# LayerXcom/zero-chain

Measured on NVIDIA H100. Metric: g1_msm_mops_2^20, higher is better.
Workload: dtype u32-limb Montgomery (Fq 12x32, Fr 8x32), integer

## Files before the change

### zero_chain_b200/csrc/msm.cuh

```cuda
#pragma once
#include <cuda_runtime.h>
#include <stdint.h>
#include "curve.cuh"
#include "curve_coop.cuh"
#include "msm_accum.cuh"
#include "tma.cuh"

namespace zkmsm {

constexpr int TILE = 131072;
constexpr int SORT_THREADS = 1024;
constexpr int COARSE_THREADS = 256;
constexpr uint32_t DIGIT_ZERO = 0xffffffffu;

static __global__ void k_msm_digits(const uint32_t *__restrict__ scalars, uint32_t n, int c, int W,
                             uint32_t *__restrict__ digits, int *__restrict__ err) {
    __shared__ __align__(128) uint4 tile[256 * 2];
    __shared__ uint64_t bar;
    uint32_t i0 = blockIdx.x * blockDim.x, i = i0 + threadIdx.x;
    uint32_t ws = blockIdx.y;
    uint32_t cnt = n - i0 < blockDim.x ? n - i0 : blockDim.x;
    if (threadIdx.x == 0) zktma::mbar_init(&bar, 1);
    __syncthreads();
    if (threadIdx.x == 0) {
// ... 213 lines not shown
    if (threadIdx.x < nb) {
        size_t b = ((size_t)g << low) + threadIdx.x;
        sizes[b] = v;
        bucket_off[b] = r0 + excl;
        hist[threadIdx.x] = r0 + excl;
        off[threadIdx.x] = excl;
        if (threadIdx.x == nb - 1) off[nb] = excl + v;
    }
    if (cb == n_coarse - 1 && dom == (int)gridDim.y - 1 && threadIdx.x == 0) bucket_off[((size_t)g + 1) << low] = r1;
    __syncthreads();
    const uint32_t total = r1 - r0;
    if (total > (uint32_t)FINE_MAX_SEGMENTS * FINE_STAGE) {
        block_for_each<uint2, 4>(coarse_sorted + r0, total, [&](uint2 e, uint64_t) { sorted[atomicAdd(&hist[e.y & fmask], 1u)] = e.x; });
        return;
    }
    for (uint32_t lo = 0; lo < nb;) {
        const uint32_t base = off[lo];
        const int fit = __syncthreads_count(threadIdx.x >= lo && threadIdx.x < nb && off[threadIdx.x + 1] - base <= (uint32_t)FINE_STAGE);
        const uint32_t hi = lo + (fit > 0 ? (uint32_t)fit : 1u);
        const bool direct = fit == 0;
        block_for_each<uint2, 2>(coarse_sorted + r0, total, [&](uint2 e, uint64_t) {
            const uint32_t k = e.y & fmask;
            if (k >= lo && k < hi) {
                const uint32_t p = atomicAdd(&hist[k], 1u);
                if (direct) sorted[p] = e.x;
                else stage[p - r0 - base] = e.x;
            }
        });
        __syncthreads();
        if (!direct)
            for (uint32_t j = threadIdx.x, m = off[hi] - base; j < m; j += blockDim.x) sorted[r0 + base + j] = stage[j];
        __syncthreads();
        lo = hi;
    }
}

constexpr int SCAN_T = 256, SCAN_E = 8, SCAN_B = SCAN_T * SCAN_E;
template <bool TASKS>
__device__ __forceinline__ uint32_t scan_load(const uint32_t *in, size_t i, uint32_t task_len) {
    uint32_t v = in[i];
    if (!TASKS) return v;
    if (v == 0) return 0;
    uint32_t t = (v + task_len / 2) / task_len;
    return t ? t : 1;
}
static __global__ void k_pick_task_len(const uint32_t *__restrict__ total_entries, const uint32_t *__restrict__ sorted_entries, uint32_t *__restrict__ task_len,
                                       uint32_t capacity, unsigned long long *__restrict__ work_counter, unsigned long long *__restrict__ xyzz_counter) {
    task_len[1] = 0;
    uint32_t total = *total_entries;
    *work_counter += *sorted_entries;
    *xyzz_counter += total;
    uint32_t waves = (total + (uint32_t)TASK_LEN_MAX * capacity - 1) / ((uint32_t)TASK_LEN_MAX * capacity);
    if (waves < 2) waves = 2;
    uint32_t target = (uint32_t)(0.97f * (float)waves * (float)capacity);
    uint32_t t = (total + target - 1) / (target ? target : 1);
    if (t < (uint32_t)TASK_LEN_MIN) t = TASK_LEN_MIN;
    if (t > (uint32_t)TASK_LEN_MAX + 8) t = TASK_LEN_MAX + 8;
    *task_len = t;
}
template <bool TASKS>
__global__ void __launch_bounds__(SCAN_T) k_scan_block(const uint32_t *__restrict__ in, uint32_t *__restrict__ out,
                                                       uint32_t *__restrict__ block_sums, size_t n, const uint32_t *__restrict__ task_len_p) {
    __shared__ uint32_t wsum[SCAN_T / 32];
    const uint32_t task_len = TASKS ? *task_len_p : 1u;
    size_t base = (size_t)blockIdx.x * SCAN_B + (size_t)threadIdx.x * SCAN_E;
    uint32_t v[SCAN_E], s = 0;
#pragma unroll
    for (int k = 0; k < SCAN_E; k++) { v[k] = base + k < n ? scan_load<TASKS>(in, base + k, task_len) : 0; s += v[k]; }
    uint32_t inc = s;
#pragma unroll
    for (int o = 1; o < 32; o <<= 1) { uint32_t t = __shfl_up_sync(0xffffffffu, inc, o); if ((threadIdx.x & 31) >= o) inc += t; }
    if ((threadIdx.x & 31) == 31) wsum[threadIdx.x >> 5] = inc;
    __syncthreads();
    if (threadIdx.x < 32) {
        uint32_t w = threadIdx.x < SCAN_T / 32 ? wsum[threadIdx.x] : 0, wi = w;
#pragma unroll
        for (int o = 1; o < 32; o <<= 1) { uint32_t t = __shfl_up_sync(0xffffffffu, wi, o); if (threadIdx.x >= o) wi += t; }
        if (threadIdx.x < SCAN_T / 32) wsum[threadIdx.x] = wi - w;
        if (threadIdx.x == SCAN_T / 32 - 1 && block_sums) block_sums[blockIdx.x] = wi;
    }
    __syncthreads();
    uint32_t ex = inc - s + wsum[threadIdx.x >> 5];
#pragma unroll
    for (int k = 0; k < SCAN_E; k++) { if (base + k < n) out[base + k] = ex; ex += v[k]; }
}
static __global__ void k_scan_add(uint32_t *__restrict__ out, const uint32_t *__restrict__ block_off, size_t n) {
    size_t i = (size_t)blockIdx.x * SCAN_B + threadIdx.x;
    uint32_t o = block_off[blockIdx.x];
    for (int k = 0; k < SCAN_E; k++, i += SCAN_T) if (i < n) out[i] += o;
}
template <bool TASKS>
inline void exclusive_scan(const uint32_t *in, uint32_t *out, size_t n, uint32_t *scratch, cudaStream_t st, const uint32_t *task_len_p = nullptr) {
    size_t nb = (n + SCAN_B - 1) / SCAN_B;
    if (nb == 0) nb = 1;
    uint32_t *bs = scratch;
    k_scan_block<TASKS><<<(unsigned)nb, SCAN_T, 0, st>>>(in, out, bs, n, task_len_p);
    if (nb == 1) {
        cudaMemcpyAsync(out + n, bs, 4, cudaMemcpyDeviceToDevice, st);
        return;
    }
    uint32_t *bo = scratch + nb + 1;
    exclusive_scan<false>(bs, bo, nb, bo + nb + 2, st);
    k_scan_add<<<(unsigned)nb, SCAN_T, 0, st>>>(out, bo, n);
    cudaMemcpyAsync(out + n, bo + nb, 4, cudaMemcpyDeviceToDevice, st);
}

constexpr int LEN_BINS = 256, LEN_BLOCK = 1024;
__device__ __forceinline__ uint32_t task_len_of(const uint32_t *bucket_off, const uint32_t *task_off, uint32_t b, uint32_t &nt) {
    nt = task_off[b + 1] - task_off[b];
    if (!nt) return 0;
    uint32_t size = bucket_off[b + 1] - bucket_off[b], len = (size + nt - 1) / nt;
    return len < (uint32_t)LEN_BINS ? len : (uint32_t)LEN_BINS - 1;
}
static __global__ void __launch_bounds__(LEN_BLOCK) k_len_hist(const uint32_t *__restrict__ bucket_off, const uint32_t *__restrict__ task_off,
                                                              uint32_t n_buckets, uint32_t *__restrict__ ghist) {
    __shared__ uint32_t sh[LEN_BINS];
    if (threadIdx.x < LEN_BINS) sh[threadIdx.x] = 0;
    __syncthreads();
    uint32_t b = blockIdx.x * LEN_BLOCK + threadIdx.x, nt = 0;
    if (b < n_buckets) { uint32_t len = task_len_of(bucket_off, task_off, b, nt); if (nt) atomicAdd(&sh[len], nt); }
    __syncthreads();
    if (threadIdx.x < LEN_BINS && sh[threadIdx.x]) atomicAdd(&ghist[threadIdx.x], sh[threadIdx.x]);
}
static __global__ void __launch_bounds__(LEN_BINS) k_len_scan(uint32_t *__restrict__ ghist, uint32_t *__restrict__ cursor) {
    __shared__ uint32_t sh[LEN_BINS];
    sh[threadIdx.x] = ghist[LEN_BINS - 1 - threadIdx.x];
    __syncthreads();
    if (threadIdx.x == 0) { uint32_t run = 0; for (int i = 0; i < LEN_BINS; i++) { uint32_t v = sh[i]; sh[i] = run; run += v; } }
    __syncthreads();
    cursor[LEN_BINS - 1 - threadIdx.x] = sh[threadIdx.x];
    ghist[threadIdx.x] = 0;
}
static __global__ void __launch_bounds__(LEN_BLOCK) k_len_place(const uint32_t *__restrict__ bucket_off, const uint32_t *__restrict__ task_off,
                                                               uint32_t n_buckets, uint32_t *__restrict__ cursor, uint32_t *__restrict__ order) {
    __shared__ uint32_t cnt[LEN_BINS], base[LEN_BINS];
    if (threadIdx.x < LEN_BINS) cnt[threadIdx.x] = 0;
    __syncthreads();
    uint32_t b = blockIdx.x * LEN_BLOCK + threadIdx.x, nt = 0, len = 0, local = 0;
    if (b < n_buckets) { len = task_len_of(bucket_off, task_off, b, nt); if (nt) local = atomicAdd(&cnt[len], nt); }
    __syncthreads();
    if (threadIdx.x < LEN_BINS && cnt[threadIdx.x]) base[threadIdx.x] = atomicAdd(&cursor[threadIdx.x], cnt[threadIdx.x]);
    __syncthreads();
    if (nt) {
        uint32_t pos = base[len] + local, t0 = task_off[b];
        for (uint32_t s = 0; s < nt; s++) order[pos + s] = t0 + s;
    }
}

constexpr uint32_t COMB_SERIAL_MAX = 32;
template <class F>
__global__ void __launch_bounds__(128) k_combine_serial(const XYZZ<F> *__restrict__ partials, const uint32_t *__restrict__ task_off,
                                                        uint32_t n_buckets, XYZZ<F> *__restrict__ buckets,
                                                        uint32_t *__restrict__ heavy_list, uint32_t *__restrict__ heavy_count) {
    uint32_t b = blockIdx.x * blockDim.x + threadIdx.x;
    if (b >= n_buckets) return;
    uint32_t t0 = task_off[b], t1 = task_off[b + 1];
    if (t1 - t0 > COMB_SERIAL_MAX) { heavy_list[atomicAdd(heavy_count, 1u)] = b; return; }
    XYZZ<F> acc = XYZZ<F>::inf();
    if (t1 > t0) acc = partials[t0];
    for (uint32_t t = t0 + 1; t < t1; t++) acc.add(partials[t]);
    buckets[b] = acc;
}
template <class F>
__global__ void __launch_bounds__(128) k_combine_warp(const XYZZ<F> *__restrict__ partials, const uint32_t *__restrict__ task_off,
                                                      const uint32_t *__restrict__ heavy_list, const uint32_t *__restrict__ heavy_count,
                                                      XYZZ<F> *__restrict__ buckets) {
    extern __shared__ unsigned char smraw[];
    XYZZ<F> *sm = reinterpret_cast<XYZZ<F> *>(smraw) + (threadIdx.x >> 5) * 32;
    const uint32_t lane = threadIdx.x & 31, n_warps = (gridDim.x * blockDim.x) >> 5, n_heavy = *heavy_count;
    for (uint32_t i = (blockIdx.x * blockDim.x + threadIdx.x) >> 5; i < n_heavy; i += n_warps) {
        uint32_t b = heavy_list[i], t0 = task_off[b], t1 = task_off[b + 1];
        XYZZ<F> acc = XYZZ<F>::inf();
        for (uint32_t t = t0 + lane; t < t1; t += 32) acc.add(partials[t]);
        __syncwarp();
        sm[lane] = acc;
        __syncwarp();
        for (int o = 16; o > 0; o >>= 1) {
            if (lane < (uint32_t)o) { XYZZ<F> x = sm[lane]; x.add(sm[lane + o]); sm[lane] = x; }
            __syncwarp();
        }
        if (lane == 0) buckets[b] = sm[0];
    }
}

constexpr int RED_T = 128, RED_SLICE = 512;
#ifndef ZK_RC_GL
#define ZK_RC_GL 8
#endif
constexpr int RC_GL = ZK_RC_GL;
#ifndef ZK_RC_MINB
#define ZK_RC_MINB 2
#endif
template <class F>
__device__ __forceinline__ void warp_tree(XYZZ<F> *slot, XYZZ<F> &acc, uint32_t lane) {
    slot[lane] = acc;
    __syncwarp();
    for (int o = 16; o > 0; o >>= 1) {
        if (lane < o) { XYZZ<F> x = slot[lane]; x.add(slot[lane + o]); slot[lane] = x; }
        __syncwarp();
    }
    acc = slot[0];
}
template <class F>
__global__ void __launch_bounds__(RED_T) k_bit_sums(const XYZZ<F> *__restrict__ B, int N, int n_slices, int n_bits, int n_dom,
                                                    XYZZ<F> *__restrict__ part) {
    extern __shared__ unsigned char smraw[];
    uint32_t lane = threadIdx.x & 31;
    XYZZ<F> *slot = reinterpret_cast<XYZZ<F> *>(smraw) + (threadIdx.x >> 5) * 32;
    size_t gw = ((size_t)blockIdx.x * blockDim.x + threadIdx.x) >> 5;
    if (gw >= (size_t)n_slices * n_bits * n_dom) return;
    int slice = (int)(gw % n_slices), bit = (int)((gw / n_slices) % n_bits), dom = (int)(gw / ((size_t)n_slices * n_bits));
    const XYZZ<F> *p = B + (size_t)dom * N;
    uint32_t k0 = (uint32_t)slice * (RED_SLICE / 2), k1 = k0 + RED_SLICE / 2;
    XYZZ<F> acc = XYZZ<F>::inf();
    for (uint32_t k = k0 + lane; k < k1; k += 32) {
        uint32_t d = ((k >> bit) << (bit + 1)) | (1u << bit) | (k & ((1u << bit) - 1u));
        if (d <= (uint32_t)N) acc.add(p[d - 1]);
    }
    warp_tree(slot, acc, lane);
    if (lane == 0) part[((size_t)dom * n_bits + bit) * n_slices + slice] = acc;
}
template <class F>
__global__ void __launch_bounds__(RED_T) k_sum_points(const XYZZ<F> *__restrict__ P, int N, int n_groups, XYZZ<F> *__restrict__ out) {
    extern __shared__ unsigned char smraw[];
    uint32_t lane = threadIdx.x & 31;
    XYZZ<F> *slot = reinterpret_cast<XYZZ<F> *>(smraw) + (threadIdx.x >> 5) * 32;
    size_t g = ((size_t)blockIdx.x * blockDim.x + threadIdx.x) >> 5;
    if (g >= (size_t)n_groups) return;
    const XYZZ<F> *p = P + g * N;
    XYZZ<F> acc = XYZZ<F>::inf();
    for (int j = lane; j < N; j += 32) acc.add(p[j]);
    warp_tree(slot, acc, lane);
    if (lane == 0) out[g] = acc;
}
constexpr int FIN_WARPS = 10;
template <class F>
__global__ void __launch_bounds__(FIN_WARPS * 32) k_finish_bits(const XYZZ<F> *__restrict__ X, int n_bits, int n_dom, XYZZ<F> *__restrict__ R) {
    extern __shared__ unsigned char smraw[];
    XYZZ<F> *vals = reinterpret_cast<XYZZ<F> *>(smraw);
    const int dom = blockIdx.x, w = threadIdx.x >> 5, lane = threadIdx.x & 31;
    if (dom >= n_dom) return;
    if (threadIdx.x < 2 * FIN_WARPS) vals[threadIdx.x] = (int)threadIdx.x < n_bits ? X[(size_t)dom * n_bits + threadIdx.x] : XYZZ<F>::inf();
    __syncthreads();
    for (int s = 0; (1 << s) < n_bits; s++) {
        const int step = 1 << s, i = w * 2 * step;
        if (i + step < n_bits) {
            XYZZ<F> hi = vals[i + step], v = vals[i];
            for (int k = 0; k < step; k++) zkcoop::dbl(hi);
            zkcoop::add(v, hi);
            __syncwarp();
            if (lane == 0) vals[i] = v;
        }
        __syncthreads();
    }
    if (threadIdx.x == 0) R[dom] = vals[0];
}
template <class F>
__device__ __noinline__ void add_outline(XYZZ<F> &acc, const XYZZ<F> &o) { acc.add(o); }
template <class F, int GL>
__global__ void __launch_bounds__(RED_T, (sizeof(F) == sizeof(Fq) ? ZK_RC_MINB : 1)) k_rowcol_sums(const XYZZ<F> *__restrict__ B, int N, int s, int n_dom, XYZZ<F> *__restrict__ rc) {
    extern __shared__ unsigned char smraw[];
    const uint32_t lane = threadIdx.x & 31, sub = lane & (GL - 1);
    XYZZ<F> *slot = reinterpret_cast<XYZZ<F> *>(smraw) + (threadIdx.x >> 5) * 32;
    const int S = 1 << s, nr = N >> s, nc = S - 1;
    const size_t n_items = (size_t)n_dom * (nr + nc);
    size_t item = ((((size_t)blockIdx.x * blockDim.x + threadIdx.x) >> 5) * (32 / GL)) + (lane / GL);
    const bool live = item < n_items;
    int dom = 0, idx = 0;
    XYZZ<F> acc = XYZZ<F>::inf();
    if (live) {
        dom = (int)(item / (nr + nc)); idx = (int)(item % (nr + nc));
        const XYZZ<F> *p = B + (size_t)dom * N;
        if (idx < nr) {
            int hi = idx + 1;
            for (int lo = sub; lo < S; lo += GL) { int d = hi * S + lo; if (d <= N) add_outline(acc, p[d - 1]); }
        } else {
            int lo = idx - nr + 1;
            for (int hi = sub; hi <= nr; hi += GL) { int d = hi * S + lo; if (d <= N) add_outline(acc, p[d - 1]); }
        }
    }
    slot[lane] = acc;
    __syncwarp();
    for (int o = GL / 2; o > 0; o >>= 1) {
        if (sub < (uint32_t)o) { XYZZ<F> x = slot[lane]; add_outline(x, slot[lane + o]); slot[lane] = x; }
        __syncwarp();
    }
    if (live && sub == 0) {
        if (idx < nr) rc[((size_t)2 * dom) * nr + idx] = slot[lane]; else rc[((size_t)2 * dom + 1) * nr + (idx - nr)] = slot[lane];
    }
}
constexpr int RC_L1 = 16, RC_L2 = 8;
template <class F>
__global__ void __launch_bounds__(RED_T) k_rowcol_stage1(const XYZZ<F> *__restrict__ B, int N, int s, int n_dom, int P1, XYZZ<F> *__restrict__ t1) {
    const int S = 1 << s, nr = N >> s, nc = S - 1;
    const int P1r = (S + RC_L1 - 1) / RC_L1, P1c = (nr + 1 + RC_L1 - 1) / RC_L1;
    size_t id = (size_t)blockIdx.x * blockDim.x + threadIdx.x;
    const size_t n_row = (size_t)n_dom * nr * P1r, n_col = (size_t)n_dom * nc * P1c;
    if (id >= n_row + n_col) return;
    int dom, idx, k, which;
    if (id < n_row) { which = 0; k = (int)(id % P1r); size_t q = id / P1r; idx = (int)(q % nr); dom = (int)(q / nr); }
    else { id -= n_row; which = 1; k = (int)(id % P1c); size_t q = id / P1c; idx = (int)(q % nc); dom = (int)(q / nc); }
    const XYZZ<F> *p = B + (size_t)dom * N;
    XYZZ<F> acc = XYZZ<F>::inf();
    if (which == 0) {
        int hi = idx + 1, lo1 = (k + 1) * RC_L1 < S ? (k + 1) * RC_L1 : S;
        for (int lo = k * RC_L1; lo < lo1; lo++) { int d = hi * S + lo; if (d <= N) acc.add(p[d - 1]); }
    } else {
        int lo = idx + 1, h1 = (k + 1) * RC_L1 < nr + 1 ? (k + 1) * RC_L1 : nr + 1;
        for (int hi = k * RC_L1; hi < h1; hi++) { int d = hi * S + lo; if (d <= N) acc.add(p[d - 1]); }
    }
    t1[((size_t)(2 * dom + which) * nr + idx) * P1 + k] = acc;
}
template <class F>
__global__ void __launch_bounds__(RED_T) k_seg_sums(const XYZZ<F> *__restrict__ in, size_t n_groups, int P_in, int L, int P_out, XYZZ<F> *__restrict__ out) {
    size_t id = (size_t)blockIdx.x * blockDim.x + threadIdx.x;
    if (id >= n_groups * P_out) return;
    const size_t g = id / P_out; const int k = (int)(id % P_out);
    const XYZZ<F> *p = in + g * P_in;
    int j1 = (k + 1) * L < P_in ? (k + 1) * L : P_in;
    XYZZ<F> acc = XYZZ<F>::inf();
    for (int j = k * L; j < j1; j++) acc.add(p[j]);
    out[id] = acc;
}
template <class F>
__global__ void __launch_bounds__(128) k_join_rowcol(const XYZZ<F> *__restrict__ Rrc, int s, int n_dom, XYZZ<F> *__restrict__ R) {
    int dom = (blockIdx.x * blockDim.x + threadIdx.x) >> 5;
    if (dom >= n_dom) return;
    XYZZ<F> r = Rrc[2 * dom];
    for (int k = 0; k < s; k++) zkcoop::dbl(r);
    zkcoop::add(r, Rrc[2 * dom + 1]);
    if ((threadIdx.x & 31) == 0) R[dom] = r;
}

template <class F>
__global__ void __launch_bounds__(32) k_horner_windows(const XYZZ<F> *__restrict__ R, int W, int c, XYZZ<F> *__restrict__ out) {
    XYZZ<F> r = R[W - 1];
    for (int w = W - 2; w >= 0; w--) {
        for (int k = 0; k < c; k++) zkcoop::dbl(r);
        zkcoop::add(r, R[w]);
    }
    if (threadIdx.x == 0) out[0] = r;
}

constexpr int PRE_K = 4;
template <class F>
__global__ void __launch_bounds__(128) k_precompute(Affine<F> *__restrict__ tbl, uint32_t n, int c, int W) {
    uint32_t i0 = (blockIdx.x * blockDim.x + threadIdx.x) * PRE_K;
    if (i0 >= n) return;
    int m = n - i0 < PRE_K ? n - i0 : PRE_K;
    for (int w = 1; w < W; w++) {
        XYZZ<F> q[PRE_K];
        F pre[PRE_K];
        F accz = F::one();
        for (int k = 0; k < m; k++) {
            Affine<F> a = tbl[(size_t)(w - 1) * n + i0 + k];
            XYZZ<F> x = XYZZ<F>::dbl_affine(a);
            for (int d = 1; d < c; d++) x = x.dbl();
            q[k] = x;
            pre[k] = accz;
            if (!x.is_inf()) accz = accz * x.zzz;
        }
        F inv = accz.inverse();
        for (int k = m - 1; k >= 0; k--) {
            Affine<F> r;
            if (q[k].is_inf()) r = Affine<F>::inf();
            else {
                F zi = inv * pre[k];
                inv = inv * q[k].zzz;
                F zi2 = (zi * q[k].zz).sqr();
                r.x = q[k].x * zi2; r.y = q[k].y * zi;
            }
            tbl[(size_t)w * n + i0 + k] = r;
        }
    }
}

template <class F>
__global__ void k_to_affine(const XYZZ<F> *__restrict__ in, Affine<F> *__restrict__ out, int n) {
    int i = blockIdx.x * blockDim.x + threadIdx.x;
    if (i < n) out[i] = in[i].to_affine();
}

}
```

### zero_chain_b200/csrc/msm_affine_core.cuh

```cuda
#pragma once
#include "curve.cuh"

namespace zkmsm {

enum { PAIR_ADD = 0, PAIR_DBL = 1, PAIR_COPY0 = 2, PAIR_COPY1 = 3, PAIR_INF = 4 };

template <class F>
struct PairIO {
    const Affine<F> *pts;
    const uint32_t *sorted;
    ZK_DEV Affine<F> load(uint32_t i) const {
        Affine<F> p;
        if (sorted) {
            uint32_t code = sorted[i];
            p = pts[code & 0x7fffffffu];
            p.y = p.y.cneg(code >> 31);
        } else p = pts[i];
        return p;
    }
};

template <class F>
ZK_DEV int pair_classify(const Affine<F> &p0, const Affine<F> &p1, bool has1, F &den) {
    den = F::one();
    if (!has1 || p1.is_inf()) return PAIR_COPY0;
    if (p0.is_inf()) return PAIR_COPY1;
    if (p0.x == p1.x) {
        if (p0.y == p1.y) {
            den = p0.y.dbl();
            if (!den.is_zero()) return PAIR_DBL;
            den = F::one();
            return PAIR_INF;
        }
        return PAIR_INF;
    }
    den = p1.x - p0.x;
    return PAIR_ADD;
}
template <class F>
ZK_DEV Affine<F> pair_finish(int mode, const Affine<F> &p0, const Affine<F> &p1, const F &dinv) {
    if (mode == PAIR_COPY0) return p0;
    if (mode == PAIR_COPY1) return p1;
    if (mode == PAIR_INF) return Affine<F>::inf();
    F lam;
    if (mode == PAIR_DBL) { F xx = p0.x.sqr(); lam = (xx.dbl() + xx) * dinv; }
    else lam = (p1.y - p0.y) * dinv;
    Affine<F> r;
    r.x = lam.sqr() - p0.x - p1.x;
    r.y = lam * (p0.x - r.x) - p0.y;
    return r;
}

}
```

### zero_chain_b200/csrc/msm_batchaff.cuh

```cuda
#pragma once
#include <cuda_runtime.h>
#include <stdint.h>
#include "curve.cuh"
#include "msm_affine_core.cuh"
#include "msm_warp_scan.cuh"

namespace zkmsm {

constexpr int BA_T = 128;
constexpr int BA_K = 32;
constexpr int BA_MINB = 4;
constexpr int BA_MAX_LEVELS = 8;
constexpr int BA_INV_T = 512;
constexpr uint32_t BA_NONE = 0xffffffffu;

static __global__ void k_half_sizes(const uint32_t *__restrict__ off_in, uint32_t *__restrict__ sizes_out, uint32_t n_buckets) {
    uint32_t b = blockIdx.x * blockDim.x + threadIdx.x;
    if (b < n_buckets) sizes_out[b] = (off_in[b + 1] - off_in[b] + 1) >> 1;
}

template <class F>
__device__ __forceinline__ void ba_store_f(F *dst, const F &v) {
    const uint4 *s = reinterpret_cast<const uint4 *>(&v);
    uint4 *d = reinterpret_cast<uint4 *>(dst);
#pragma unroll
    for (int k = 0; k < (int)(sizeof(F) / 16); k++) d[k] = s[k];
}
template <class F>
__device__ __forceinline__ F ba_load_f(const F *src) {
    F v;
    const uint4 *s = reinterpret_cast<const uint4 *>(src);
    uint4 *d = reinterpret_cast<uint4 *>(&v);
#pragma unroll
    for (int k = 0; k < (int)(sizeof(F) / 16); k++) d[k] = s[k];
    return v;
}
template <class F>
__device__ __forceinline__ F ba_ldg_f(const F *src) {
    F v;
    const uint4 *s = reinterpret_cast<const uint4 *>(src);
    uint4 *d = reinterpret_cast<uint4 *>(&v);
#pragma unroll
    for (int k = 0; k < (int)(sizeof(F) / 16); k++) d[k] = __ldg(s + k);
    return v;
}
template <class F, bool FIRST>
__device__ __forceinline__ const F *ba_x(const F *in_x, uint32_t code) { return FIRST ? in_x + 2 * (size_t)(code & 0x7fffffffu) : in_x + code; }
template <class F, bool FIRST>
__device__ __forceinline__ const F *ba_y(const F *in_x, const F *in_y, uint32_t code) { return FIRST ? ba_x<F, FIRST>(in_x, code) + 1 : in_y + code; }
template <class F, bool FIRST>
__device__ __forceinline__ Affine<F> ba_load_point(const F *in_x, const F *in_y, uint32_t code) {
    Affine<F> p;
    p.x = ba_ldg_f(ba_x<F, FIRST>(in_x, code));
    p.y = ba_ldg_f(ba_y<F, FIRST>(in_x, in_y, code));
    if (FIRST) p.y = p.y.cneg(code >> 31);
    return p;
}

struct BaWalk {
    uint32_t b, out0, out1, in0, in1;
    __device__ __forceinline__ BaWalk(const uint32_t *off_in, const uint32_t *off_out, uint32_t n_buckets, uint32_t o) {
        uint32_t lo = 0, hi = n_buckets;
        while (hi - lo > 1) { uint32_t mid = (lo + hi) >> 1; if (off_out[mid] <= o) lo = mid; else hi = mid; }
        b = lo; out0 = off_out[b]; out1 = off_out[b + 1]; in0 = off_in[b]; in1 = off_in[b + 1];
    }
    __device__ __forceinline__ void forward(const uint32_t *off_in, const uint32_t *off_out, uint32_t o) {
        while (o >= out1) { b++; out0 = out1; out1 = off_out[b + 1]; in0 = in1; in1 = off_in[b + 1]; }
    }
    __device__ __forceinline__ void backward(const uint32_t *off_in, const uint32_t *off_out, uint32_t o) {
        while (o < out0) { b--; out1 = out0; out0 = off_out[b]; in1 = in0; in0 = off_in[b]; }
    }
    template <bool FIRST>
    __device__ __forceinline__ uint2 src(const uint32_t *sorted, uint32_t o) const {
        const uint32_t i0 = in0 + 2 * (o - out0);
        uint2 s;
        s.x = FIRST ? sorted[i0] : i0;
        s.y = i0 + 1 < in1 ? (FIRST ? sorted[i0 + 1] : i0 + 1) : BA_NONE;
        return s;
    }
};
__device__ __forceinline__ uint32_t ba_lane_first(size_t tid, int K) { return (uint32_t)(tid >> 5) * 32u * (uint32_t)K + (uint32_t)(tid & 31); }
__device__ __forceinline__ int ba_lane_count(uint32_t total, uint32_t oa, int K) {
    if (oa >= total) return 0;
    const uint32_t n = (total - oa + 31) >> 5;
    return n < (uint32_t)K ? (int)n : K;
}

template <class F, bool FIRST>
__global__ void __launch_bounds__(BA_T, 4) k_ba_forward(const F *__restrict__ in_x, const F *__restrict__ in_y, const uint32_t *__restrict__ sorted,
                                                         const uint32_t *__restrict__ off_in, const uint32_t *__restrict__ off_out, uint32_t n_buckets, int K,
                                                         F *__restrict__ prefix, F *__restrict__ block_totals) {
    const uint32_t total = off_out[n_buckets];
    const uint32_t n_blocks = (total + BA_T * K - 1) / (BA_T * K);
    if (blockIdx.x >= n_blocks) return;
    const int t = threadIdx.x;
    const size_t T_total = (size_t)gridDim.x * BA_T, tid = (size_t)blockIdx.x * BA_T + t;
    const uint32_t oa = ba_lane_first(tid, K);
    const int n = ba_lane_count(total, oa, K);
    F run = F::one();
    if (n > 0) {
        BaWalk w(off_in, off_out, n_buckets, oa);
        uint2 s0 = w.src<FIRST>(sorted, oa), s1 = make_uint2(0, BA_NONE);
        F xa0 = ba_ldg_f(ba_x<F, FIRST>(in_x, s0.x)), xa1 = s0.y != BA_NONE ? ba_ldg_f(ba_x<F, FIRST>(in_x, s0.y)) : F::zero();
        F xb0 = F::zero(), xb1 = F::zero();
        if (n > 1) {
            w.forward(off_in, off_out, oa + 32);
            s1 = w.src<FIRST>(sorted, oa + 32);
            xb0 = ba_ldg_f(ba_x<F, FIRST>(in_x, s1.x));
            if (s1.y != BA_NONE) xb1 = ba_ldg_f(ba_x<F, FIRST>(in_x, s1.y));
        }
        for (int k = 0; k < n; k++) {
            const uint2 cur = s0;
            const F x0 = xa0, x1 = xa1;
            s0 = s1; xa0 = xb0; xa1 = xb1;
            if (k + 2 < n) {
                const uint32_t o = oa + 32u * (uint32_t)(k + 2);
                w.forward(off_in, off_out, o);
                s1 = w.src<FIRST>(sorted, o);
                xb0 = ba_ldg_f(ba_x<F, FIRST>(in_x, s1.x));
                if (s1.y != BA_NONE) xb1 = ba_ldg_f(ba_x<F, FIRST>(in_x, s1.y));
            }
            ba_store_f(prefix + (size_t)k * T_total + tid, run);
            if (cur.y == BA_NONE) continue;
            F den = x1 - x0;
            if (den.is_zero() || x0.is_zero() || x1.is_zero()) {
                Affine<F> p0 = ba_load_point<F, FIRST>(in_x, in_y, cur.x), p1 = ba_load_point<F, FIRST>(in_x, in_y, cur.y);
                if (pair_classify(p0, p1, true, den) > PAIR_DBL) continue;
            }
            run = run * den;
        }
    }
    F others, all;
    ba_warp_products(run, others, all);
    ba_store_f(prefix + (size_t)K * T_total + tid, others);
    if ((t & 31) == 0) ba_store_f(block_totals + (tid >> 5), all);
}

template <class F>
__global__ void __launch_bounds__(BA_INV_T) k_ba_invert(const F *__restrict__ totals, const uint32_t *__restrict__ off_out, uint32_t n_buckets, int K,
                                                        F *__restrict__ scratch, F *__restrict__ inv_out) {
    extern __shared__ unsigned char ba_smem[];
    F *node = reinterpret_cast<F *>(ba_smem);
    const uint32_t total = off_out[n_buckets];
    const uint32_t n = ((total + BA_T * K - 1) / (BA_T * K)) * (BA_T / 32);
    const int t = threadIdx.x;
    const uint32_t per = (n + BA_INV_T - 1) / BA_INV_T, c0 = t * per, c1 = c0 + per < n ? c0 + per : n;
    F run = F::one();
    for (uint32_t i = c0; i < c1; i++) { ba_store_f(scratch + i, run); run = run * ba_load_f(totals + i); }
    node[BA_INV_T + t] = run;
    for (int s = BA_INV_T / 2; s >= 1; s >>= 1) {
        __syncthreads();
        if (t < s) node[s + t] = node[2 * (s + t)] * node[2 * (s + t) + 1];
    }
    __syncthreads();
    if (t == 0) node[1] = node[1].inverse();
    for (int s = 1; s < BA_INV_T; s <<= 1) {
        __syncthreads();
        if (t < s) {
            F inv = node[s + t], l = node[2 * (s + t)], r = node[2 * (s + t) + 1];
            node[2 * (s + t)] = inv * r;
            node[2 * (s + t) + 1] = inv * l;
        }
    }
    __syncthreads();
    F inv = node[BA_INV_T + t];
    for (uint32_t i = c1; i-- > c0;) {
        F v = ba_load_f(totals + i);
        ba_store_f(inv_out + i, inv * ba_load_f(scratch + i));
        inv = inv * v;
    }
}

template <class F, bool FIRST, int MINB>
__global__ void __launch_bounds__(BA_T, MINB) k_ba_backward(const F *__restrict__ in_x, const F *__restrict__ in_y, const uint32_t *__restrict__ sorted,
                                                             const uint32_t *__restrict__ off_in, const uint32_t *__restrict__ off_out, uint32_t n_buckets, int K,
                                                             const F *__restrict__ prefix, const F *__restrict__ block_inv,
                                                             F *__restrict__ out_x, F *__restrict__ out_y) {
    constexpr int PV = (int)(sizeof(Affine<F>) / 16), FV = (int)(sizeof(F) / 16);
    extern __shared__ unsigned char ba_smem[];
    uint4 *stage = reinterpret_cast<uint4 *>(ba_smem);
    const uint32_t total = off_out[n_buckets];
    const uint32_t n_blocks = (total + BA_T * K - 1) / (BA_T * K);
    if (blockIdx.x >= n_blocks) return;
    const int t = threadIdx.x;
    const size_t T_total = (size_t)gridDim.x * BA_T, tid = (size_t)blockIdx.x * BA_T + t;
    const uint32_t oa = ba_lane_first(tid, K);
    const int n = ba_lane_count(total, oa, K);
    if (n == 0) return;
    F inv = ba_load_f(block_inv + (tid >> 5)) * ba_load_f(prefix + (size_t)K * T_total + tid);
    uint4 *slot = stage + t;
    auto copy = [&](int v, const F *src) {
        const uint4 *s = reinterpret_cast<const uint4 *>(src);
#pragma unroll
        for (int u = 0; u < FV; u++)
            asm volatile("cp.async.cg.shared.global [%0], [%1], 16;" ::"r"((uint32_t)__cvta_generic_to_shared(slot + (v + u) * BA_T)), "l"(s + u) : "memory");
    };
    auto prefetch = [&](int k, uint2 src) {
        const uint32_t c1 = src.y == BA_NONE ? src.x : src.y;
        copy(0, ba_x<F, FIRST>(in_x, src.x));
        copy(FV, ba_y<F, FIRST>(in_x, in_y, src.x));
        copy(PV, ba_x<F, FIRST>(in_x, c1));
        copy(PV + FV, ba_y<F, FIRST>(in_x, in_y, c1));
        copy(2 * PV, prefix + (size_t)k * T_total + tid);
        asm volatile("cp.async.commit_group;" ::: "memory");
    };
    BaWalk w(off_in, off_out, n_buckets, oa + 32u * (uint32_t)(n - 1));
    uint2 src = w.src<FIRST>(sorted, oa + 32u * (uint32_t)(n - 1));
    prefetch(n - 1, src);
    for (int k = n; k-- > 0;) {
        asm volatile("cp.async.wait_group 0;" ::: "memory");
        Affine<F> p0, p1;
        F pre;
        {
            uint4 *d0 = reinterpret_cast<uint4 *>(&p0), *d1 = reinterpret_cast<uint4 *>(&p1), *d2 = reinterpret_cast<uint4 *>(&pre);
#pragma unroll
            for (int v = 0; v < PV; v++) { d0[v] = slot[v * BA_T]; d1[v] = slot[(PV + v) * BA_T]; }
#pragma unroll
            for (int v = 0; v < FV; v++) d2[v] = slot[(2 * PV + v) * BA_T];
        }
        const uint2 cur = src;
        if (k > 0) {
            const uint32_t o = oa + 32u * (uint32_t)(k - 1);
            w.backward(off_in, off_out, o);
            src = w.src<FIRST>(sorted, o);
            prefetch(k - 1, src);
        }
        const bool has1 = cur.y != BA_NONE;
        if (FIRST) { p0.y = p0.y.cneg(cur.x >> 31); if (has1) p1.y = p1.y.cneg(cur.y >> 31); }
        if (!has1) p1 = Affine<F>::inf();
        F den;
        const int mode = pair_classify(p0, p1, has1, den);
        F dinv = F::one();
        if (mode <= PAIR_DBL) { dinv = inv * pre; inv = inv * den; }
        Affine<F> r = pair_finish(mode, p0, p1, dinv);
        const uint32_t o = oa + 32u * (uint32_t)k;
        ba_store_f(out_x + o, r.x);
        ba_store_f(out_y + o, r.y);
    }
}

template <class F> constexpr size_t ba_smem_forward() { return 0; }
template <class F> constexpr size_t ba_smem_backward() { return (size_t)BA_T * (2 * sizeof(Affine<F>) + sizeof(F)); }
template <class F> constexpr size_t ba_smem_invert() { return 2 * BA_INV_T * sizeof(F); }

}
```

### zero_chain_b200/csrc/msm_driver.cuh

```cuda
#pragma once
#include "internal.h"
#include "msm.cuh"
#include "msm_batchaff.cuh"
#include "codec.cuh"
#include <stdlib.h>

namespace zkmsm {

template <class F>
int build_tables_t(zk_ctx *ctx, zk_bases *b) {
    unsigned thr = 128, blk = (unsigned)((b->n + thr * PRE_K - 1) / (thr * PRE_K));
    k_precompute<F><<<blk, thr, 0, ctx->stream>>>((Affine<F> *)b->d_tbl, (uint32_t)b->n, b->c, b->W);
    ZK_CUDA(cudaGetLastError());
    return ZK_OK;
}

template <class F>
int msm_run_t(zk_ctx *ctx, const zk_bases *b, const uint32_t *d_scalars, size_t n, size_t batch) {
    cudaStream_t st = ctx->stream;
    const int c = b->c, W = b->W, nbins = 1 << (c - 1);
    const bool tables = b->tables;
    if (!tables && batch != 1) { zk_set_error("batched MSM needs precomputed tables"); return ZK_ERR_INVALID; }
    const size_t n_dom = tables ? batch : (size_t)W;
    const uint64_t e_dom = tables ? (uint64_t)n * W : (uint64_t)n;
    const size_t E = (size_t)n * W * batch;
    if (E >= ((size_t)1 << 31)) { zk_set_error("MSM too large for 31-bit entry payloads (n*W*batch = %zu)", E); return ZK_ERR_INVALID; }
    const bool two_level = c > 16;
    const int low = two_level ? (c - 1) - 9 : 0, sort_bins = two_level ? 512 : nbins;
    size_t smem = (size_t)sort_bins * 4;
    uint32_t tile_len = TILE;
    if (two_level) {
        int per_sm = 0;
        ZK_CUDA(cudaOccupancyMaxActiveBlocksPerMultiprocessor(&per_sm, k_coarse_scatter, COARSE_THREADS, 0));
        tile_len = coarse_tile_len(e_dom, n_dom, per_sm * ctx->sm_count);
    }
    const int tiles = (int)((e_dom + tile_len - 1) / tile_len);
    const size_t NB = n_dom * nbins;
    size_t t_max = E / TASK_LEN_MAX + 2 * (size_t)ctx->sm_count * 1024u + 1;
    t_max += NB + 1;
    const size_t pt = sizeof(XYZZ<F>);
    ZK_TRY(ctx->digits.reserve(E * 4));
    ZK_TRY(ctx->tile_hist.reserve(n_dom * tiles * (size_t)(c > 16 ? 512 : nbins) * 4));
    ZK_TRY(ctx->tile_off.reserve(n_dom * tiles * (size_t)(c > 16 ? 512 : nbins) * 4));
    ZK_TRY(ctx->sizes.reserve((NB + 1) * 4));
    ZK_TRY(ctx->bucket_off.reserve((NB + 1) * 4));
    ZK_TRY(ctx->task_off.reserve((NB + 1) * 4));
    ZK_TRY(ctx->scan_scratch.reserve((2 * (NB / SCAN_B + 8) + 4096) * 4));
    ZK_TRY(ctx->sorted.reserve(E * 4));
    ZK_TRY(ctx->partials.reserve(t_max * pt));
    ZK_TRY(ctx->buckets.reserve(NB * pt));
    const int n_bits = c;
    const int n_slices = (nbins / 2 + RED_SLICE / 2 - 1) / (RED_SLICE / 2) > 0 ? (nbins / 2 + RED_SLICE / 2 - 1) / (RED_SLICE / 2) : 1;
    ZK_TRY(ctx->red_part.reserve(2 * n_dom * n_bits * (size_t)n_slices * pt));
    ZK_TRY(ctx->red_x.reserve(2 * n_dom * n_bits * pt));
    ZK_TRY(ctx->result.reserve((n_dom + batch + 1) * pt));

    uint32_t *digits = ctx->digits.as<uint32_t>();
    {
        dim3 g((unsigned)((n + 255) / 256), (unsigned)batch);
        k_msm_digits<<<g, 256, 0, st>>>(d_scalars, (uint32_t)n, c, W, digits, ctx->d_err);
    }
    const size_t SB = n_dom * (size_t)sort_bins;
    if (smem > 48 * 1024) {
        ZK_CUDA(cudaFuncSetAttribute(k_tile_hist, cudaFuncAttributeMaxDynamicSharedMemorySize, (int)smem));
        ZK_CUDA(cudaFuncSetAttribute(k_scatter, cudaFuncAttributeMaxDynamicSharedMemorySize, (int)smem));
    }
    dim3 gs((unsigned)tiles, (unsigned)n_dom);
    if (!two_level) {
        k_tile_hist<<<gs, SORT_THREADS, smem, st>>>(digits, e_dom, nbins, 0, ctx->tile_hist.as<uint32_t>(), tiles, tile_len, false);
        k_col_scan<<<(unsigned)((NB + 255) / 256), 256, 0, st>>>(ctx->tile_hist.as<uint32_t>(), ctx->tile_off.as<uint32_t>(), ctx->sizes.as<uint32_t>(),
                                                                nbins, tiles, (int)n_dom);
        exclusive_scan<false>(ctx->sizes.as<uint32_t>(), ctx->bucket_off.as<uint32_t>(), NB, ctx->scan_scratch.as<uint32_t>(), st);
        k_scatter<<<gs, SORT_THREADS, smem, st>>>(digits, e_dom, nbins, ctx->tile_off.as<uint32_t>(), ctx->bucket_off.as<uint32_t>(),
                                                  ctx->sorted.as<uint32_t>(), tiles, tile_len);
    } else {
        ZK_TRY(ctx->sorted2.reserve(E * sizeof(uint2)));
        ZK_TRY(ctx->coarse_off.reserve((SB + 1) * 4)); ZK_TRY(ctx->coarse_sizes.reserve((SB + 1) * 4));
        k_tile_hist<<<gs, COARSE_THREADS, smem, st>>>(digits, e_dom, sort_bins, low, ctx->tile_hist.as<uint32_t>(), tiles, tile_len, true);
        k_bin_scan<<<(unsigned)SB, COARSE_THREADS, 0, st>>>(ctx->tile_hist.as<uint32_t>(), ctx->tile_off.as<uint32_t>(), ctx->coarse_sizes.as<uint32_t>(), tiles);
        exclusive_scan<false>(ctx->coarse_sizes.as<uint32_t>(), ctx->coarse_off.as<uint32_t>(), SB, ctx->scan_scratch.as<uint32_t>(), st);
        k_coarse_scatter<<<gs, COARSE_THREADS, 0, st>>>(digits, e_dom, low, ctx->tile_off.as<uint32_t>(), ctx->coarse_off.as<uint32_t>(),
                                                        ctx->sorted2.as<uint2>(), tiles, tile_len);
        ZK_CUDA(cudaFuncSetAttribute(k_fine_sort, cudaFuncAttributeMaxDynamicSharedMemorySize, FINE_STAGE * 4));
        k_fine_sort<<<dim3(512, (unsigned)n_dom), 1024, FINE_STAGE * 4, st>>>(ctx->sorted2.as<uint2>(), ctx->coarse_off.as<uint32_t>(), 512, low,
                                                                 ctx->sizes.as<uint32_t>(), ctx->bucket_off.as<uint32_t>(), ctx->sorted.as<uint32_t>());
    }
    const F *cur_x = (const F *)b->d_tbl, *cur_y = nullptr;
    const uint32_t *cur_sorted = ctx->sorted.as<uint32_t>(), *cur_off = ctx->bucket_off.as<uint32_t>(), *cur_sizes = ctx->sizes.as<uint32_t>();
    struct ProfPair {
        cudaEvent_t a = nullptr, b = nullptr; bool kept = false;
        ~ProfPair() { if (!kept) { if (a) cudaEventDestroy(a); if (b) cudaEventDestroy(b); } }
    } prof;
    cudaEvent_t &ev0 = prof.a, &ev1 = prof.b;
    {
        int levels = 0;
        if (ctx->opts.ba_min_entries >= 0 && (long)E >= ctx->opts.ba_min_entries) {
            if (ctx->opts.ba_levels >= 0) levels = (int)(ctx->opts.ba_levels < BA_MAX_LEVELS ? ctx->opts.ba_levels : BA_MAX_LEVELS);
            else for (size_t avg = E / NB; avg >= 12 && levels < BA_MAX_LEVELS; avg >>= 1) levels++;
        }
        if (ctx->prof_on && levels > 0) { cudaEventCreate(&ev0); cudaEventCreate(&ev1); cudaEventRecord(ev0, st); }
        size_t in_max = E;
        int minb = BA_MINB, k_force = 0;
        (void)minb;
#ifdef ZK_EXPERIMENTS
        if (const char *e = getenv("ZK_BA_MINB")) minb = atoi(e);
        if (const char *e = getenv("ZK_BA_K")) k_force = atoi(e);
#endif
        DevBuf *pts_buf[2] = {&ctx->aff_pts0, &ctx->aff_pts1}, *off_buf[2] = {&ctx->aff_off0, &ctx->aff_off1}, *sz_buf[2] = {&ctx->aff_sizes0, &ctx->aff_sizes1};
        if (levels > 0) {
            if (ba_smem_backward<F>() > 48 * 1024) {
                ZK_CUDA(cudaFuncSetAttribute(k_ba_backward<F, true, BA_MINB>, cudaFuncAttributeMaxDynamicSharedMemorySize, (int)ba_smem_backward<F>()));
                ZK_CUDA(cudaFuncSetAttribute(k_ba_backward<F, false, BA_MINB>, cudaFuncAttributeMaxDynamicSharedMemorySize, (int)ba_smem_backward<F>()));
#ifdef ZK_EXPERIMENTS
                ZK_CUDA(cudaFuncSetAttribute(k_ba_backward<F, true, 3>, cudaFuncAttributeMaxDynamicSharedMemorySize, (int)ba_smem_backward<F>()));
                ZK_CUDA(cudaFuncSetAttribute(k_ba_backward<F, false, 3>, cudaFuncAttributeMaxDynamicSharedMemorySize, (int)ba_smem_backward<F>()));
#endif
            }
            if (ba_smem_invert<F>() > 48 * 1024)
                ZK_CUDA(cudaFuncSetAttribute(k_ba_invert<F>, cudaFuncAttributeMaxDynamicSharedMemorySize, (int)ba_smem_invert<F>()));
        }
        for (int l = 0; l < levels; l++) {
            const size_t out_max = (in_max + NB) / 2 + 1;
            int K = BA_K;
            if (k_force > 0) K = k_force;
            const unsigned grid = (unsigned)((out_max + (size_t)BA_T * K - 1) / ((size_t)BA_T * K));
            const size_t T_total = (size_t)grid * BA_T;
            DevBuf *pts_o = pts_buf[l & 1], *off_o = off_buf[l & 1], *sz_o = sz_buf[l & 1];
            ZK_TRY(pts_o->reserve(out_max * sizeof(Affine<F>)));
            F *out_x = pts_o->as<F>(), *out_y = out_x + out_max;
            ZK_TRY(off_o->reserve((NB + 1) * 4)); ZK_TRY(sz_o->reserve((NB + 1) * 4));
            ZK_TRY(ctx->aff_scratch.reserve((size_t)(K + 1) * T_total * sizeof(F)));
            const size_t n_tot = (size_t)grid * (BA_T / 32);
            ZK_TRY(ctx->aff_tot.reserve(3 * n_tot * sizeof(F)));
            F *tot = ctx->aff_tot.as<F>(), *tot_scr = tot + n_tot, *tot_inv = tot + 2 * n_tot;
            k_half_sizes<<<(unsigned)((NB + 255) / 256), 256, 0, st>>>(cur_off, sz_o->as<uint32_t>(), (uint32_t)NB);
            exclusive_scan<false>(sz_o->as<uint32_t>(), off_o->as<uint32_t>(), NB, ctx->scan_scratch.as<uint32_t>(), st);
            const uint32_t *off_out = off_o->as<uint32_t>();
            if (l == 0)
                k_ba_forward<F, true><<<grid, BA_T, ba_smem_forward<F>(), st>>>(cur_x, cur_y, cur_sorted, cur_off, off_out, (uint32_t)NB, K, ctx->aff_scratch.as<F>(), tot);
            else
                k_ba_forward<F, false><<<grid, BA_T, ba_smem_forward<F>(), st>>>(cur_x, cur_y, nullptr, cur_off, off_out, (uint32_t)NB, K, ctx->aff_scratch.as<F>(), tot);
            k_ba_invert<F><<<1, BA_INV_T, ba_smem_invert<F>(), st>>>(tot, off_out, (uint32_t)NB, K, tot_scr, tot_inv);
            const int Kb = K;
#define ZK_BA_BWD(FIRST_, MB_) k_ba_backward<F, FIRST_, MB_><<<grid, BA_T, ba_smem_backward<F>(), st>>>(cur_x, cur_y, cur_sorted, cur_off, off_out, (uint32_t)NB, Kb, \
                                                                                                    ctx->aff_scratch.as<F>(), tot_inv, out_x, out_y)
#ifdef ZK_EXPERIMENTS
            if (minb == 3) { if (l == 0) ZK_BA_BWD(true, 3); else ZK_BA_BWD(false, 3); } else
#endif
            { if (l == 0) ZK_BA_BWD(true, BA_MINB); else ZK_BA_BWD(false, BA_MINB); }
#undef ZK_BA_BWD
            cur_x = out_x; cur_y = out_y; cur_sorted = nullptr;
            cur_off = off_out; cur_sizes = sz_o->as<uint32_t>();
            in_max = out_max;
        }
    }
    uint32_t *d_task_len = (uint32_t *)(ctx->d_err + 8);
    const uint32_t capacity = (uint32_t)ctx->sm_count * 3u * 128u;
    unsigned long long *d_work = (unsigned long long *)(ctx->d_err + (sizeof(F) == sizeof(Fq) ? 10 : 12));
    k_pick_task_len<<<1, 1, 0, st>>>(cur_off + NB, ctx->bucket_off.as<uint32_t>() + NB, d_task_len, capacity, d_work, d_work + 2);
    exclusive_scan<true>(cur_sizes, ctx->task_off.as<uint32_t>(), NB, ctx->scan_scratch.as<uint32_t>(), st, d_task_len);
    XYZZ<F> *partials = ctx->partials.as<XYZZ<F>>(), *buckets = ctx->buckets.as<XYZZ<F>>();
    const uint32_t *order = nullptr;
    {
        bool want = E / NB < 256;
        if (want) {
            ZK_TRY(ctx->task_order.reserve(t_max * 4)); ZK_TRY(ctx->len_hist.reserve(2 * LEN_BINS * 4 + 64));
            uint32_t *gh = ctx->len_hist.as<uint32_t>(), *cur = gh + LEN_BINS;
            if (!ctx->len_hist_zeroed) { ZK_CUDA(cudaMemsetAsync(gh, 0, 2 * LEN_BINS * 4, st)); ctx->len_hist_zeroed = true; }
            unsigned nb = (unsigned)((NB + LEN_BLOCK - 1) / LEN_BLOCK);
            k_len_hist<<<nb, LEN_BLOCK, 0, st>>>(cur_off, ctx->task_off.as<uint32_t>(), (uint32_t)NB, gh);
            k_len_scan<<<1, LEN_BINS, 0, st>>>(gh, cur);
            k_len_place<<<nb, LEN_BLOCK, 0, st>>>(cur_off, ctx->task_off.as<uint32_t>(), (uint32_t)NB, cur, ctx->task_order.as<uint32_t>());
            order = ctx->task_order.as<uint32_t>();
        }
    }
    {
        const uint32_t *so = cur_sorted, *bo = cur_off, *to = ctx->task_off.as<uint32_t>();
        unsigned grid = (unsigned)((t_max + 127) / 128);
        if (ctx->prof_on && !ev0) { cudaEventCreate(&ev0); cudaEventCreate(&ev1); cudaEventRecord(ev0, st); }
        k_accumulate<F, 3><<<grid, 128, 0, st>>>(cur_x, cur_y, so, bo, to, (uint32_t)NB, order, partials);
    }
    if (ctx->prof_on) { cudaEventRecord(ev1, st); ctx->prof_events.push_back(ev0); ctx->prof_events.push_back(ev1); prof.kept = true; }
    if (ctx->split_tail) {
        ZK_CUDA(cudaEventRecord(ctx->ev_front, st));
        ZK_CUDA(cudaStreamWaitEvent(ctx->tail, ctx->ev_front, 0));
        st = ctx->tail;
    }
    const size_t sm_warp = 4 * 32 * pt;
    if (sm_warp > 48 * 1024) {
        ZK_CUDA(cudaFuncSetAttribute(k_combine_warp<F>, cudaFuncAttributeMaxDynamicSharedMemorySize, (int)sm_warp));
        ZK_CUDA(cudaFuncSetAttribute(k_bit_sums<F>, cudaFuncAttributeMaxDynamicSharedMemorySize, (int)sm_warp));
        ZK_CUDA(cudaFuncSetAttribute(k_sum_points<F>, cudaFuncAttributeMaxDynamicSharedMemorySize, (int)sm_warp));
        ZK_CUDA(cudaFuncSetAttribute(k_finish_bits<F>, cudaFuncAttributeMaxDynamicSharedMemorySize, (int)sm_warp));
    }
    ZK_TRY(ctx->heavy_list.reserve((NB + 1) * 4));
    uint32_t *heavy_count = d_task_len + 1;
    k_combine_serial<F><<<(unsigned)((NB + 127) / 128), 128, 0, st>>>(partials, ctx->task_off.as<uint32_t>(), (uint32_t)NB, buckets,
                                                                      ctx->heavy_list.as<uint32_t>(), heavy_count);
    k_combine_warp<F><<<(unsigned)(2 * ctx->sm_count), 128, sm_warp, st>>>(partials, ctx->task_off.as<uint32_t>(), ctx->heavy_list.as<uint32_t>(), heavy_count, buckets);
    XYZZ<F> *part = ctx->red_part.as<XYZZ<F>>(), *X = ctx->red_x.as<XYZZ<F>>(), *R = ctx->result.as<XYZZ<F>>();
    auto bit_reduce = [&](const XYZZ<F> *Bk, int N, int bits, size_t nd, XYZZ<F> *out) {
        int slices = (N / 2 + RED_SLICE / 2 - 1) / (RED_SLICE / 2); if (slices < 1) slices = 1;
        size_t n_w = (size_t)slices * bits * nd, n_g = nd * (size_t)bits;
        k_bit_sums<F><<<(unsigned)((n_w * 32 + RED_T - 1) / RED_T), RED_T, sm_warp, st>>>(Bk, N, slices, bits, (int)nd, part);
        k_sum_points<F><<<(unsigned)((n_g * 32 + RED_T - 1) / RED_T), RED_T, sm_warp, st>>>(part, slices, (int)n_g, X);
        k_finish_bits<F><<<(unsigned)nd, FIN_WARPS * 32, 2 * FIN_WARPS * sizeof(XYZZ<F>), st>>>(X, bits, (int)nd, out);
    };
    XYZZ<F> *Rdom = tables ? R : R + 1;
    if ((n_dom >= 8 && c >= 7) || (tables && c > 16)) {
        const int s = (c - 1) / 2, nr = nbins >> s, nc = (1 << s) - 1;
        ZK_TRY(ctx->red_rows.reserve(2 * n_dom * (size_t)nr * pt));
        ZK_TRY(ctx->result.reserve((3 * n_dom + batch + 4) * pt));
        R = ctx->result.as<XYZZ<F>>();
        Rdom = tables ? R : R + 1;
        XYZZ<F> *rc = ctx->red_rows.as<XYZZ<F>>(), *Rrc = R + n_dom + 2;
        if (sm_warp > 48 * 1024) {
            ZK_CUDA(cudaFuncSetAttribute(k_rowcol_sums<F, RC_GL>, cudaFuncAttributeMaxDynamicSharedMemorySize, (int)sm_warp));
        }
        size_t n_items = n_dom * (size_t)(nr + nc);
        if (n_dom >= 8) {
            ZK_CUDA(cudaMemsetAsync(rc, 0, 2 * n_dom * (size_t)nr * pt, st));
            constexpr int per_warp = 32 / RC_GL;
            k_rowcol_sums<F, RC_GL><<<(unsigned)((((n_items + per_warp - 1) / per_warp) * 32 + RED_T - 1) / RED_T), RED_T, sm_warp, st>>>(buckets, nbins, s, (int)n_dom, rc);
        } else {
            const size_t n_slots = 2 * n_dom * (size_t)nr;
            const int longest = (1 << s) > nr + 1 ? (1 << s) : nr + 1;
            const int P1 = (longest + RC_L1 - 1) / RC_L1, P2 = (P1 + RC_L2 - 1) / RC_L2;
            ZK_TRY(ctx->red_tmp.reserve(n_slots * (size_t)(P1 + P2) * pt));
            XYZZ<F> *t1 = ctx->red_tmp.as<XYZZ<F>>(), *t2 = t1 + n_slots * P1;
            const int P1r = ((1 << s) + RC_L1 - 1) / RC_L1, P1c = (nr + 1 + RC_L1 - 1) / RC_L1;
            const size_t live = n_dom * ((size_t)nr * P1r + (size_t)nc * P1c);
            ZK_CUDA(cudaMemsetAsync(t1, 0, n_slots * (size_t)P1 * pt, st));
            k_rowcol_stage1<F><<<(unsigned)((live + RED_T - 1) / RED_T), RED_T, 0, st>>>(buckets, nbins, s, (int)n_dom, P1, t1);
            k_seg_sums<F><<<(unsigned)((n_slots * P2 + RED_T - 1) / RED_T), RED_T, 0, st>>>(t1, n_slots, P1, RC_L2, P2, t2);
            k_seg_sums<F><<<(unsigned)((n_slots + RED_T - 1) / RED_T), RED_T, 0, st>>>(t2, n_slots, P2, P2, 1, rc);
        }
        bit_reduce(rc, nr, c - s, 2 * n_dom, Rrc);
        k_join_rowcol<F><<<(unsigned)((n_dom * 32 + 127) / 128), 128, 0, st>>>(Rrc, s, (int)n_dom, Rdom);
    } else {
        bit_reduce(buckets, nbins, n_bits, n_dom, Rdom);
    }
    if (!tables) k_horner_windows<F><<<1, 32, 0, st>>>(Rdom, W, c, R);
    ZK_CUDA(cudaGetLastError());
    return ZK_OK;
}

template <class F>
int encode_results_t(zk_ctx *ctx, size_t count, int compressed, uint8_t *d_out) {
    zkcodec::k_encode_xyzz<F><<<(unsigned)((count + 31) / 32), 32, 0, ctx->stream>>>(ctx->result.as<XYZZ<F>>(), (int)count, compressed, d_out);
    ZK_CUDA(cudaGetLastError());
    return ZK_OK;
}

}
```

Before: 165.6.

## Park pair source indices in forward pass for Fq batch-affine backward

For the Fq field, the forward batch-affine kernel now saves each step's source-index pair to scratch. The backward kernel reads these pairs directly instead of re-walking bucket offsets and re-reading the sorted array, and prefetches one step ahead. pair_finish for Fq also moves the doubling numerator into a noinline cold helper and merges the two lambda multiplies to cut code size and register pressure. The row/col stage1 loop is unified into a single strided loop. The cost is extra scratch memory and additional global stores and loads of uint2 per step.

```diff
diff --git a/zero_chain_b200/csrc/msm.cuh b/zero_chain_b200/csrc/msm.cuh
--- a/zero_chain_b200/csrc/msm.cuh
+++ b/zero_chain_b200/csrc/msm.cuh
@@ -539,13 +539,10 @@
     else { id -= n_row; which = 1; k = (int)(id % P1c); size_t q = id / P1c; idx = (int)(q % nc); dom = (int)(q / nc); }
     const XYZZ<F> *p = B + (size_t)dom * N;
     XYZZ<F> acc = XYZZ<F>::inf();
-    if (which == 0) {
-        int hi = idx + 1, lo1 = (k + 1) * RC_L1 < S ? (k + 1) * RC_L1 : S;
-        for (int lo = k * RC_L1; lo < lo1; lo++) { int d = hi * S + lo; if (d <= N) acc.add(p[d - 1]); }
-    } else {
-        int lo = idx + 1, h1 = (k + 1) * RC_L1 < nr + 1 ? (k + 1) * RC_L1 : nr + 1;
-        for (int hi = k * RC_L1; hi < h1; hi++) { int d = hi * S + lo; if (d <= N) acc.add(p[d - 1]); }
-    }
+    int d, step, m;
+    if (which == 0) { const int lo0 = k * RC_L1, lo1 = lo0 + RC_L1 < S ? lo0 + RC_L1 : S; d = (idx + 1) * S + lo0; step = 1; m = lo1 - lo0; }
+    else { const int h0 = k * RC_L1, h1 = h0 + RC_L1 < nr + 1 ? h0 + RC_L1 : nr + 1; d = h0 * S + idx + 1; step = S; m = h1 - h0; }
+    for (int j = 0; j < m; j++, d += step) if (d <= N) acc.add(p[d - 1]);
     t1[((size_t)(2 * dom + which) * nr + idx) * P1 + k] = acc;
 }
 template <class F>
diff --git a/zero_chain_b200/csrc/msm_affine_core.cuh b/zero_chain_b200/csrc/msm_affine_core.cuh
--- a/zero_chain_b200/csrc/msm_affine_core.cuh
+++ b/zero_chain_b200/csrc/msm_affine_core.cuh
@@ -37,13 +37,21 @@
     den = p1.x - p0.x;
     return PAIR_ADD;
 }
+#ifdef ZK_HOST_EMUL
+#define ZK_PAIR_COLD inline
+#else
+#define ZK_PAIR_COLD __device__ __noinline__
+#endif
+template <class F>
+ZK_PAIR_COLD F pair_dbl_num(const F x) { F xx = x.sqr(); return xx.dbl() + xx; }
 template <class F>
 ZK_DEV Affine<F> pair_finish(int mode, const Affine<F> &p0, const Affine<F> &p1, const F &dinv) {
     if (mode == PAIR_COPY0) return p0;
     if (mode == PAIR_COPY1) return p1;
     if (mode == PAIR_INF) return Affine<F>::inf();
     F lam;
-    if (mode == PAIR_DBL) { F xx = p0.x.sqr(); lam = (xx.dbl() + xx) * dinv; }
+    if (sizeof(F) == sizeof(Fq)) lam = (mode == PAIR_DBL ? pair_dbl_num(p0.x) : p1.y - p0.y) * dinv;
+    else if (mode == PAIR_DBL) { F xx = p0.x.sqr(); lam = (xx.dbl() + xx) * dinv; }
     else lam = (p1.y - p0.y) * dinv;
     Affine<F> r;
     r.x = lam.sqr() - p0.x - p1.x;
diff --git a/zero_chain_b200/csrc/msm_batchaff.cuh b/zero_chain_b200/csrc/msm_batchaff.cuh
--- a/zero_chain_b200/csrc/msm_batchaff.cuh
+++ b/zero_chain_b200/csrc/msm_batchaff.cuh
@@ -79,6 +79,8 @@
         return s;
     }
 };
+template <class F> __host__ __device__ constexpr bool ba_parks_pairs() { return sizeof(F) == sizeof(Fq); }
+
 __device__ __forceinline__ uint32_t ba_lane_first(size_t tid, int K) { return (uint32_t)(tid >> 5) * 32u * (uint32_t)K + (uint32_t)(tid & 31); }
 __device__ __forceinline__ int ba_lane_count(uint32_t total, uint32_t oa, int K) {
     if (oa >= total) return 0;
@@ -89,7 +91,7 @@
 template <class F, bool FIRST>
 __global__ void __launch_bounds__(BA_T, 4) k_ba_forward(const F *__restrict__ in_x, const F *__restrict__ in_y, const uint32_t *__restrict__ sorted,
                                                          const uint32_t *__restrict__ off_in, const uint32_t *__restrict__ off_out, uint32_t n_buckets, int K,
-                                                         F *__restrict__ prefix, F *__restrict__ block_totals) {
+                                                         F *__restrict__ prefix, uint2 *__restrict__ srcs, F *__restrict__ block_totals) {
     const uint32_t total = off_out[n_buckets];
     const uint32_t n_blocks = (total + BA_T * K - 1) / (BA_T * K);
     if (blockIdx.x >= n_blocks) return;
@@ -121,6 +123,7 @@
                 if (s1.y != BA_NONE) xb1 = ba_ldg_f(ba_x<F, FIRST>(in_x, s1.y));
             }
             ba_store_f(prefix + (size_t)k * T_total + tid, run);
+            if (ba_parks_pairs<F>()) srcs[(size_t)k * T_total + tid] = cur;
             if (cur.y == BA_NONE) continue;
             F den = x1 - x0;
             if (den.is_zero() || x0.is_zero() || x1.is_zero()) {
@@ -173,7 +176,8 @@
 
 template <class F, bool FIRST, int MINB>
 __global__ void __launch_bounds__(BA_T, MINB) k_ba_backward(const F *__restrict__ in_x, const F *__restrict__ in_y, const uint32_t *__restrict__ sorted,
-                                                             const uint32_t *__restrict__ off_in, const uint32_t *__restrict__ off_out, uint32_t n_buckets, int K,
+                                                             const uint2 *__restrict__ srcs, const uint32_t *__restrict__ off_in,
+                                                             const uint32_t *__restrict__ off_out, uint32_t n_buckets, int K,
                                                              const F *__restrict__ prefix, const F *__restrict__ block_inv,
                                                              F *__restrict__ out_x, F *__restrict__ out_y) {
     constexpr int PV = (int)(sizeof(Affine<F>) / 16), FV = (int)(sizeof(F) / 16);
@@ -204,9 +208,17 @@
         copy(2 * PV, prefix + (size_t)k * T_total + tid);
         asm volatile("cp.async.commit_group;" ::: "memory");
     };
+    constexpr bool PARKED = ba_parks_pairs<F>();
     BaWalk w(off_in, off_out, n_buckets, oa + 32u * (uint32_t)(n - 1));
-    uint2 src = w.src<FIRST>(sorted, oa + 32u * (uint32_t)(n - 1));
+    auto pair_of = [&](int k) -> uint2 {
+        if (PARKED) return srcs[(size_t)k * T_total + tid];
+        const uint32_t o = oa + 32u * (uint32_t)k;
+        w.backward(off_in, off_out, o);
+        return w.src<FIRST>(sorted, o);
+    };
+    uint2 src = pair_of(n - 1), nxt = src;
     prefetch(n - 1, src);
+    if (PARKED && n > 1) nxt = pair_of(n - 2);
     for (int k = n; k-- > 0;) {
         asm volatile("cp.async.wait_group 0;" ::: "memory");
         Affine<F> p0, p1;
@@ -220,10 +232,10 @@
         }
         const uint2 cur = src;
         if (k > 0) {
-            const uint32_t o = oa + 32u * (uint32_t)(k - 1);
-            w.backward(off_in, off_out, o);
-            src = w.src<FIRST>(sorted, o);
-            prefetch(k - 1, src);
+            if (!PARKED) nxt = pair_of(k - 1);
+            prefetch(k - 1, nxt);
+            src = nxt;
+            if (PARKED && k > 1) nxt = pair_of(k - 2);
         }
         const bool has1 = cur.y != BA_NONE;
         if (FIRST) { p0.y = p0.y.cneg(cur.x >> 31); if (has1) p1.y = p1.y.cneg(cur.y >> 31); }
diff --git a/zero_chain_b200/csrc/msm_driver.cuh b/zero_chain_b200/csrc/msm_driver.cuh
--- a/zero_chain_b200/csrc/msm_driver.cuh
+++ b/zero_chain_b200/csrc/msm_driver.cuh
@@ -129,7 +129,8 @@
             ZK_TRY(pts_o->reserve(out_max * sizeof(Affine<F>)));
             F *out_x = pts_o->as<F>(), *out_y = out_x + out_max;
             ZK_TRY(off_o->reserve((NB + 1) * 4)); ZK_TRY(sz_o->reserve((NB + 1) * 4));
-            ZK_TRY(ctx->aff_scratch.reserve((size_t)(K + 1) * T_total * sizeof(F)));
+            ZK_TRY(ctx->aff_scratch.reserve((size_t)(K + 1) * T_total * sizeof(F) + (ba_parks_pairs<F>() ? (size_t)K * T_total * sizeof(uint2) : 0)));
+            uint2 *srcs = reinterpret_cast<uint2 *>(ctx->aff_scratch.as<F>() + (size_t)(K + 1) * T_total);
             const size_t n_tot = (size_t)grid * (BA_T / 32);
             ZK_TRY(ctx->aff_tot.reserve(3 * n_tot * sizeof(F)));
             F *tot = ctx->aff_tot.as<F>(), *tot_scr = tot + n_tot, *tot_inv = tot + 2 * n_tot;
@@ -137,12 +138,12 @@
             exclusive_scan<false>(sz_o->as<uint32_t>(), off_o->as<uint32_t>(), NB, ctx->scan_scratch.as<uint32_t>(), st);
             const uint32_t *off_out = off_o->as<uint32_t>();
             if (l == 0)
-                k_ba_forward<F, true><<<grid, BA_T, ba_smem_forward<F>(), st>>>(cur_x, cur_y, cur_sorted, cur_off, off_out, (uint32_t)NB, K, ctx->aff_scratch.as<F>(), tot);
+                k_ba_forward<F, true><<<grid, BA_T, ba_smem_forward<F>(), st>>>(cur_x, cur_y, cur_sorted, cur_off, off_out, (uint32_t)NB, K, ctx->aff_scratch.as<F>(), srcs, tot);
             else
-                k_ba_forward<F, false><<<grid, BA_T, ba_smem_forward<F>(), st>>>(cur_x, cur_y, nullptr, cur_off, off_out, (uint32_t)NB, K, ctx->aff_scratch.as<F>(), tot);
+                k_ba_forward<F, false><<<grid, BA_T, ba_smem_forward<F>(), st>>>(cur_x, cur_y, nullptr, cur_off, off_out, (uint32_t)NB, K, ctx->aff_scratch.as<F>(), srcs, tot);
             k_ba_invert<F><<<1, BA_INV_T, ba_smem_invert<F>(), st>>>(tot, off_out, (uint32_t)NB, K, tot_scr, tot_inv);
             const int Kb = K;
-#define ZK_BA_BWD(FIRST_, MB_) k_ba_backward<F, FIRST_, MB_><<<grid, BA_T, ba_smem_backward<F>(), st>>>(cur_x, cur_y, cur_sorted, cur_off, off_out, (uint32_t)NB, Kb, \
+#define ZK_BA_BWD(FIRST_, MB_) k_ba_backward<F, FIRST_, MB_><<<grid, BA_T, ba_smem_backward<F>(), st>>>(cur_x, cur_y, cur_sorted, srcs, cur_off, off_out, (uint32_t)NB, Kb, \
                                                                                                     ctx->aff_scratch.as<F>(), tot_inv, out_x, out_y)
 #ifdef ZK_EXPERIMENTS
             if (minb == 3) { if (l == 0) ZK_BA_BWD(true, 3); else ZK_BA_BWD(false, 3); } else
```

Result: faster. 168.3 (median of 6 runs) (+1.7%).
